# mkkellogg/GaussianSplats3D

Measured on AMD Instinct MI355X. Metric: Msplats/s sorted+rasterized at 1920x1080 SH-2, higher is better.
Workload: dtype int32 keys / f32 raster; 1 GPU; C3: garden.ply stand-in, SH2, 1920x1080; splats=5800000, sh_degree=2, width=1920, height=1080, cull=off (R=N), sort_precision_bits=16, streams=one (SURVEY.md 8d: sort -> draw on a single stream), parallelism=1 GPU, sort=full list (R = N)

## Files before the change

### gaussiansplats3d_amd/csrc/draw_plan.cpp

```cpp
#include "draw_plan.hpp"

#include "bin_word.hpp"

#include <math.h>
#include <string.h>

#include <algorithm>

DrawFeedback read_feedback(const volatile uint32_t* mirror) {
    DrawFeedback f = {};
    if (!mirror) return f;
    f.view_serial = mirror[GS_MIRROR_VIEW_SERIAL];
    f.visible = mirror[GS_MIRROR_VISIBLE];
    const uint32_t t_lo = mirror[GS_MIRROR_TILES16_LO], t_hi = mirror[GS_MIRROR_TILES16_HI];
    f.tiles16 = ((uint64_t)t_hi << 32) | t_lo;
    f.view_valid = f.view_serial != 0u && mirror[GS_MIRROR_VIEW_SERIAL] == f.view_serial;
    f.serial = mirror[GS_MIRROR_SERIAL];
    f.overflow = mirror[GS_MIRROR_OVERFLOW] != 0u;
    const uint32_t e_lo = mirror[GS_MIRROR_ENTRIES_LO], e_hi = mirror[GS_MIRROR_ENTRIES_HI];
    f.entries = ((uint64_t)e_hi << 32) | e_lo;
    f.entries_valid = mirror[GS_MIRROR_SERIAL] == f.serial;
    f.deep_candidates = mirror[GS_MIRROR_DEEP_CANDIDATES];
    f.deep_share = mirror[GS_MIRROR_DEEP_SHARE];
    return f;
}

uint32_t adapt_list_shift(uint32_t current, uint64_t tiles16, uint32_t visible) {
    if (visible == 0u) return current;
    const float tiles = (float)tiles16, vis = (float)visible;
    static const uint32_t shifts[4] = {GS_LIST_SHIFT_SMALL, GS_LIST_SHIFT_LARGE, GS_LIST_SHIFT_BIG, GS_LIST_SHIFT_HUGE};
    static const float thr[3] = {GS_LIST_TILES_PER_SPLAT, GS_LIST_TILES_PER_SPLAT_BIG, GS_LIST_TILES_PER_SPLAT_HUGE};
    uint32_t level = 0;
    while (level < 3u && shifts[level] != current) level++;
    while (level < 3u && tiles >= 1.08f * thr[level] * vis) level++;
    while (level > 0u && tiles < 0.92f * thr[level - 1u] * vis) level--;
    return shifts[level];
}

int block_test_mode(uint32_t measured_visible, uint32_t measured_count, bool strip, bool block_cull, bool no_block_list, bool block_test_always) {
    const bool measured = measured_count > 0u;
    const bool all_live = measured && (uint64_t)measured_visible * 10u > (uint64_t)measured_count * 9u;
    const bool half_live = measured && !all_live && (uint64_t)measured_visible * 20u > (uint64_t)measured_count * 11u;
    const bool test = block_cull && (!all_live || strip || block_test_always);
    const bool pretest = test && !no_block_list && (!half_live || strip || block_test_always);
    return pretest ? 1 : (test ? 0 : 2);
}

bool narrow_bin_word(uint32_t tiles_x, uint32_t tiles_y, const DrawSwitches& sw) {
    return tiles_x <= BIN_WORD_NARROW_TILES && tiles_y <= BIN_WORD_NARROW_TILES && !sw.no_compact_bin_word;
}

SchedulePlan plan_schedule(const ScheduleInputs& in) {
    const DrawSwitches& sw = in.sw;
    const PlanView& pp = in.now;
    SchedulePlan plan = {};
    const uint32_t blend_bins = in.bins_x * (in.bin_row_end - in.bin_row_begin);
    plan.blend_bins = blend_bins;
    plan.deep_factor = sw.deep_factor;
    plan.deep_min = in.draw_mode == GS_DRAW_FP32 ? sw.deep_min : 0x7FFFFFFFu;
    const bool order_ok = blend_bins > 0 && blend_bins <= 8192u && in.stats.bins == blend_bins && in.stats.row_begin == in.bin_row_begin &&
                          in.stats.width_px == (uint32_t)pp.width && in.stats.draw_mode == in.draw_mode && !sw.no_blend_order;
    plan.order_ok = order_ok;
    const PlanView& lp = in.stats.view;
    const bool same_frame = in.stats.valid && memcmp(lp.proj, pp.proj, sizeof(pp.proj)) == 0 && lp.width == pp.width && lp.height == pp.height &&
                            lp.count == pp.count && lp.list_shift == pp.list_shift;
    bool same_view = same_frame && memcmp(lp.view, pp.view, sizeof(pp.view)) == 0;
    if (same_frame && !same_view && in.block_cull && in.centre_n > 0) {
        const float limit = sw.order_motion;
        const double inv_n = 1.0 / (double)in.centre_n;
        const float c[3] = {(float)(in.centre_sum[0] * inv_n), (float)(in.centre_sum[1] * inv_n), (float)(in.centre_sum[2] * inv_n)};
        auto window = [&](const PlanView& q, const float* p, float* xy) {
            float v[4], o[4];
            for (int r = 0; r < 4; r++) v[r] = q.view[r] * p[0] + q.view[4 + r] * p[1] + q.view[8 + r] * p[2] + q.view[12 + r];
            for (int r = 0; r < 4; r++) o[r] = q.proj[r] * v[0] + q.proj[4 + r] * v[1] + q.proj[8 + r] * v[2] + q.proj[12 + r] * v[3];
            if (!(o[3] > 1e-6f)) return false;
            xy[0] = (o[0] / o[3] * 0.5f + 0.5f) * q.width;
            xy[1] = (o[1] / o[3] * 0.5f + 0.5f) * q.height;
            return true;
        };
        float was[2], is[2];
        if (window(lp, c, was) && window(pp, c, is)) {
            const float dx = (is[0] - was[0]) / (float)GS_BIN, dy = (is[1] - was[1]) / (float)GS_BIN;
            const bool shift_ok = fabsf(dx) < 4096.0f && fabsf(dy) < 4096.0f && !sw.no_stat_shift;
            if (shift_ok) {
                plan.sx = (int32_t)lrintf(dx);
                plan.sy = (int32_t)lrintf(dy);
            }
            const float* V = lp.view;
            const float a00 = V[0], a10 = V[1], a20 = V[2], a01 = V[4], a11 = V[5], a21 = V[6], a02 = V[8], a12 = V[9], a22 = V[10];
            const float c00 = a11 * a22 - a12 * a21, c01 = a02 * a21 - a01 * a22, c02 = a01 * a12 - a02 * a11;
            const float det = a00 * c00 + a10 * c01 + a20 * c02;
            const float b0 = V[12], b1 = V[13], b2 = V[14], id = 1.0f / det;
            const float eye[3] = {-(c00 * b0 + c01 * b1 + c02 * b2) * id,
                                  -((a12 * a20 - a10 * a22) * b0 + (a00 * a22 - a02 * a20) * b1 + (a02 * a10 - a00 * a12) * b2) * id,
                                  -((a10 * a21 - a11 * a20) * b0 + (a01 * a20 - a00 * a21) * b1 + (a00 * a11 - a01 * a10) * b2) * id};
            float parallax = 0.0f;
            bool seen = fabsf(det) > 1e-20f;
            for (int k = 0; k < 2 && seen; k++) {
                const float t = k ? 2.0f : 0.5f;
                const float p[3] = {eye[0] + t * (c[0] - eye[0]), eye[1] + t * (c[1] - eye[1]), eye[2] + t * (c[2] - eye[2])};
                float at[2];
                seen = window(pp, p, at);
                if (seen) parallax = fmaxf(parallax, sqrtf((at[0] - is[0]) * (at[0] - is[0]) + (at[1] - is[1]) * (at[1] - is[1])));
            }
            const float moved = (parallax + (shift_ok ? 0.0f : sqrtf(dx * dx + dy * dy) * (float)GS_BIN)) / fmaxf(pp.height, 1.0f);
            same_view = seen && moved <= limit;
        }
    }
    plan.same_view = same_view;
    const bool stale_order = sw.blend_order_stale;
    plan.deep_pass = order_ok && in.draw_mode == GS_DRAW_FP32 && !in.no_deep && in.feedback.deep_candidates > 0u;
    plan.order_wg = order_ok && (same_view || stale_order || plan.deep_pass || pp.list_shift == GS_LIST_SHIFT_SMALL || (in.draw_serial & 7u) == 7u);
    plan.order_taken = order_ok && (same_view || stale_order || (plan.deep_pass && !sw.deep_row_major_on_motion));
    return plan;
}

constexpr float DEEP_WGS_PER_SHARE = 0.6f;

DeepUnits place_deep_units(const SchedulePlan& plan, uint32_t bins, uint32_t cu_count, uint32_t occupancy, const DrawFeedback& feedback,
                           const DrawSwitches& sw) {
    DeepUnits du;
    du.unit_wgs = plan.deep_pass ? cu_count * occupancy : 0u;
    du.unit_at = bins;
    if (plan.deep_pass && plan.order_taken && !sw.deep_units_last) {
        const uint32_t cus = cu_count;
        const uint32_t deep_hint = feedback.deep_candidates;
        const float share = (float)std::min(feedback.deep_share, 1024u) * (1.0f / 1024.0f);
        const float k = DEEP_WGS_PER_SHARE;
        du.unit_wgs = std::min(du.unit_wgs, std::max(2u * cus, (uint32_t)(k * share * (float)du.unit_wgs + 0.5f)));
        du.unit_at = std::min(bins, std::min(deep_hint, (uint32_t)GS_DEEP_MAX_BINS) + cus + cus / 2u);
    }
    return du;
}

static PlanView plan_view(const float* view, const float* proj, float width, float height, uint32_t count, uint32_t list_shift) {
    PlanView v;
    memcpy(v.view, view, sizeof(v.view));
    memcpy(v.proj, proj, sizeof(v.proj));
    v.width = width; v.height = height; v.count = count; v.list_shift = list_shift;
    return v;
}

extern "C" int gs_debug_draw_plan(const gs_draw_plan_debug_in* in, gs_draw_plan_debug_out* out) {
    if (!in || !out) return -1;
    const DrawFeedback fb = read_feedback(in->mirror);
    ScheduleInputs si = {};
    si.stats.valid = in->stats_valid != 0u;
    si.stats.bins = in->stats_bins; si.stats.row_begin = in->stats_row_begin; si.stats.width_px = in->stats_width_px; si.stats.draw_mode = in->stats_mode;
    si.stats.view = plan_view(in->stats_view, in->stats_proj, in->stats_width, in->stats_height, in->stats_count, in->stats_list_shift);
    si.now = plan_view(in->view, in->proj, in->width, in->height, in->count, in->list_shift);
    si.bins_x = in->bins_x; si.bin_row_begin = in->bin_row_begin; si.bin_row_end = in->bin_row_end;
    si.block_cull = in->block_cull; si.draw_mode = in->draw_mode; si.draw_serial = in->draw_serial; si.no_deep = in->no_deep != 0u;
    memcpy(si.centre_sum, in->centre_sum, sizeof(si.centre_sum));
    si.centre_n = in->centre_n;
    si.feedback = fb;
    si.sw.deep_min = in->deep_min; si.sw.deep_factor = in->deep_factor; si.sw.no_blend_order = in->no_blend_order != 0u;
    si.sw.order_motion = in->order_motion; si.sw.no_stat_shift = in->no_stat_shift != 0u; si.sw.blend_order_stale = in->blend_order_stale != 0u;
    si.sw.deep_row_major_on_motion = in->deep_row_major_on_motion != 0u; si.sw.deep_units_last = in->deep_units_last != 0u;
    const SchedulePlan plan = plan_schedule(si);
    const DeepUnits du = place_deep_units(plan, plan.blend_bins, in->cu_count, in->occupancy, fb, si.sw);
    *out = gs_draw_plan_debug_out();
    out->entries = fb.entries; out->tiles16 = fb.tiles16; out->room = entry_room(in->need);
    out->entries_valid = fb.entries_valid; out->serial = fb.serial; out->overflow = fb.overflow;
    out->deep_candidates = fb.deep_candidates; out->deep_share = fb.deep_share;
    out->view_valid = fb.view_valid; out->view_serial = fb.view_serial; out->visible = fb.visible;
    out->blend_bins = plan.blend_bins; out->order_ok = plan.order_ok; out->same_view = plan.same_view;
    out->sx = plan.sx; out->sy = plan.sy;
    out->order_wg = plan.order_wg; out->order_taken = plan.order_taken; out->deep_pass = plan.deep_pass;
    out->deep_min = plan.deep_min; out->deep_factor = plan.deep_factor;
    out->unit_at = du.unit_at; out->unit_wgs = du.unit_wgs;
    out->list_shift = adapt_list_shift(in->list_current, in->tiles16, in->visible);
    out->block_test = block_test_mode(in->measured_visible, in->measured_count, in->strip != 0u, in->block_cull != 0u, in->no_block_list != 0u,
                                      in->block_test_always != 0u);
    return 0;
}

extern "C" int gs_debug_bin_word(const gs_bin_word_debug_in* in, gs_bin_word_debug_out* out) {
    if (!in || !out) return -1;
    DrawSwitches sw = {};
    sw.no_compact_bin_word = in->no_compact_bin_word != 0u;
    *out = gs_bin_word_debug_out();
    out->narrow = narrow_bin_word(in->tiles_x, in->tiles_y, sw) ? 1u : 0u;
    const BinRect r = {in->x0 | (in->y0 << 16), in->x1 | (in->y1 << 16)};
    out->word = bin_word_pack_narrow(in->visible != 0u, in->slot, r);
    const BinWordOut n = bin_word_unpack_narrow(out->word);
    out->visible = n.visible; out->escape = n.escape; out->slot = n.slot;
    if (n.visible && !n.escape) { out->x0 = n.rect.lo & 0xFFFFu; out->y0 = n.rect.lo >> 16; out->x1 = n.rect.hi & 0xFFFFu; out->y1 = n.rect.hi >> 16; }
    const BinWordWide w = bin_word_pack_wide(in->visible != 0u, in->slot, r);
    out->wide_lo = w.x; out->wide_hi = w.y;
    const BinWordOut u = bin_word_unpack_wide(w);
    out->wide_visible = u.visible; out->wide_slot = u.slot;
    out->wide_x0 = u.rect.lo & 0xFFFFu; out->wide_y0 = u.rect.lo >> 16; out->wide_x1 = u.rect.hi & 0xFFFFu; out->wide_y1 = u.rect.hi >> 16;
    return 0;
}
```

### gaussiansplats3d_amd/csrc/draw_plan.hpp

```cpp
#pragma once
#include <stdint.h>

#include "../../include/gsplat_hip.h"

constexpr uint32_t GS_BIN_SHIFT = 1;
constexpr uint32_t GS_BIN = GS_TILE << GS_BIN_SHIFT;
constexpr uint32_t GS_LIST_SHIFT_LARGE = 3;
constexpr uint32_t GS_LIST_SHIFT_SMALL = GS_BIN_SHIFT;
constexpr float GS_LIST_TILES_PER_SPLAT = 3.0f;
constexpr uint32_t GS_LIST_SHIFT_BIG = 4, GS_LIST_SHIFT_HUGE = 5;
constexpr float GS_LIST_TILES_PER_SPLAT_BIG = 21.0f, GS_LIST_TILES_PER_SPLAT_HUGE = 80.0f;
constexpr uint32_t GS_DEEP_MAX_BINS = 512;

constexpr uint32_t GS_MIRROR_SERIAL = 0, GS_MIRROR_OVERFLOW = 1, GS_MIRROR_ENTRIES_LO = 2, GS_MIRROR_ENTRIES_HI = 3;
constexpr uint32_t GS_MIRROR_DEEP_CANDIDATES = 4, GS_MIRROR_DEEP_SHARE = 5;
constexpr uint32_t GS_MIRROR_VIEW_SERIAL = 8, GS_MIRROR_VISIBLE = 9, GS_MIRROR_TILES16_LO = 10, GS_MIRROR_TILES16_HI = 11;
constexpr uint32_t GS_MIRROR_WORDS = 16;
static_assert(GS_MIRROR_SERIAL % 4 == 0 && GS_MIRROR_OVERFLOW == GS_MIRROR_SERIAL + 1 && GS_MIRROR_ENTRIES_LO == GS_MIRROR_SERIAL + 2 &&
              GS_MIRROR_ENTRIES_HI == GS_MIRROR_SERIAL + 3, "k_bin_emit writes the verdict as one aligned 16-byte store");
static_assert(GS_MIRROR_VIEW_SERIAL % 4 == 0 && GS_MIRROR_VISIBLE == GS_MIRROR_VIEW_SERIAL + 1 && GS_MIRROR_TILES16_LO == GS_MIRROR_VIEW_SERIAL + 2 &&
              GS_MIRROR_TILES16_HI == GS_MIRROR_VIEW_SERIAL + 3, "k_bin_emit writes the view share as one aligned 16-byte store");

struct DrawFeedback {
    bool entries_valid;
    uint32_t serial;
    bool overflow;
    uint64_t entries;
    uint32_t deep_candidates;
    uint32_t deep_share;
    bool view_valid;
    uint32_t view_serial, visible;
    uint64_t tiles16;
};
DrawFeedback read_feedback(const volatile uint32_t* mirror);

struct DrawSwitches {
    uint32_t deep_min;
    uint32_t deep_factor;
    uint32_t pool_slots;
    bool no_lazy_mask;
    bool no_blend_order;
    float order_motion;
    bool no_stat_shift;
    bool blend_order_stale;
    bool deep_row_major_on_motion;
    bool no_async_list_bins;
    bool deep_units_last;
    bool no_compact_bin_word;
};

uint32_t adapt_list_shift(uint32_t current, uint64_t tiles16, uint32_t visible);

inline uint64_t entry_room(uint64_t need) { return need + need / 8 + 1024; }

int block_test_mode(uint32_t measured_visible, uint32_t measured_count, bool strip, bool block_cull, bool no_block_list, bool block_test_always);

bool narrow_bin_word(uint32_t tiles_x, uint32_t tiles_y, const DrawSwitches& sw);

struct PlanView {
    float view[16], proj[16];
    float width, height;
    uint32_t count, list_shift;
};
struct StatsOf {
    bool valid;
    uint32_t bins, row_begin, width_px;
    uint32_t draw_mode;
    PlanView view;
};
struct ScheduleInputs {
    StatsOf stats;
    PlanView now;
    uint32_t bins_x, bin_row_begin, bin_row_end;
    uint32_t block_cull;
    uint32_t draw_mode;
    uint32_t draw_serial;
    bool no_deep;
    double centre_sum[3];
    uint64_t centre_n;
    DrawFeedback feedback;
    DrawSwitches sw;
};
struct SchedulePlan {
    uint32_t blend_bins;
    bool order_ok;
    bool same_view;
    int32_t sx, sy;
    bool order_wg;
    bool order_taken;
    bool deep_pass;
    uint32_t deep_min, deep_factor;
};
SchedulePlan plan_schedule(const ScheduleInputs& in);

struct DeepUnits { uint32_t unit_at, unit_wgs; };
DeepUnits place_deep_units(const SchedulePlan& plan, uint32_t bins, uint32_t cu_count, uint32_t occupancy, const DrawFeedback& feedback,
                           const DrawSwitches& sw);

struct gs_draw_plan_debug_in {
    double centre_sum[3];
    uint64_t centre_n;
    uint64_t tiles16;
    uint64_t need;
    uint32_t mirror[GS_MIRROR_WORDS];
    uint32_t stats_valid, stats_bins, stats_row_begin, stats_width_px, stats_mode;
    float stats_view[16], stats_proj[16], stats_width, stats_height;
    uint32_t stats_count, stats_list_shift;
    float view[16], proj[16], width, height;
    uint32_t count, list_shift, bins_x, bin_row_begin, bin_row_end, block_cull, draw_mode, draw_serial, no_deep;
    uint32_t deep_min, deep_factor, no_blend_order;
    float order_motion;
    uint32_t no_stat_shift, blend_order_stale, deep_row_major_on_motion, deep_units_last;
    uint32_t cu_count, occupancy;
    uint32_t list_current, visible;
    uint32_t measured_visible, measured_count, strip, no_block_list, block_test_always;
};
struct gs_draw_plan_debug_out {
    uint64_t entries, tiles16, room;
    uint32_t entries_valid, serial, overflow, deep_candidates, deep_share, view_valid, view_serial, visible;
    uint32_t blend_bins, order_ok, same_view;
    int32_t sx, sy;
    uint32_t order_wg, order_taken, deep_pass, deep_min, deep_factor;
    uint32_t unit_at, unit_wgs, list_shift;
    int32_t block_test;
};
extern "C" int gs_debug_draw_plan(const gs_draw_plan_debug_in* in, gs_draw_plan_debug_out* out);

struct gs_bin_word_debug_in {
    uint32_t tiles_x, tiles_y, no_compact_bin_word;
    uint32_t visible, slot, x0, y0, x1, y1;
};
struct gs_bin_word_debug_out {
    uint32_t narrow;
    uint32_t word;
    uint32_t visible, escape, slot, x0, y0, x1, y1;
    uint32_t wide_lo, wide_hi;
    uint32_t wide_visible, wide_slot, wide_x0, wide_y0, wide_x1, wide_y1;
};
extern "C" int gs_debug_bin_word(const gs_bin_word_debug_in* in, gs_bin_word_debug_out* out);
```

### gaussiansplats3d_amd/csrc/tile_bin.hip

```cpp
#include <stdlib.h>

#include "radix.hpp"

constexpr int BIN_THREADS = 256;
#ifndef BIN_PER_LANE
#define BIN_PER_LANE 4
#endif
#ifndef BIN_MAX_BLOCKS_CFG
#define BIN_MAX_BLOCKS_CFG 2048
#endif
constexpr int BIN_MAX_BLOCKS = BIN_MAX_BLOCKS_CFG;
constexpr uint32_t ANY_WORDS = 2048;

__device__ __forceinline__ uint32_t rect_tiles(uint2 r) {
    const uint32_t x0 = r.x & 0xFFFFu, y0 = r.x >> 16, x1 = r.y & 0xFFFFu, y1 = r.y >> 16;
    return (x1 >= x0 && y1 >= y0) ? (x1 - x0 + 1u) * (y1 - y0 + 1u) : 0u;
}
__device__ __forceinline__ uint2 rect_to_bins(uint2 r, uint32_t list_shift) {
    const uint32_t field = 0xFFFFu >> list_shift, mask = field | (field << 16);
    return make_uint2((r.x >> list_shift) & mask, (r.y >> list_shift) & mask);
}

struct BinChunk {
    uint32_t begin, end;
    uint32_t id;
};
__device__ __forceinline__ BinChunk bin_chunk(uint32_t n) {
    const uint32_t batches = (n + BIN_THREADS - 1) / BIN_THREADS;
    const uint32_t per = (batches + gridDim.x - 1) / gridDim.x;
    BinChunk c;
    c.id = xcd_chunk(blockIdx.x, gridDim.x);
    c.begin = min(c.id * per, batches);
    c.end = min(c.begin + per, batches);
    return c;
}

#ifdef GS_BIN_PROFILE
__device__ unsigned long long g_bin_prof[2 * 2048 * 4];
extern "C" int gs_debug_bin_prof(void* dst) {
    return (int)hipMemcpyFromSymbol(dst, HIP_SYMBOL(g_bin_prof), sizeof(unsigned long long) * 2 * 2048 * 4, 0, hipMemcpyDeviceToHost);
}
#define BIN_PROF(k, slot, v) do { if (threadIdx.x == 0 && blockIdx.x < 2048u) g_bin_prof[((k) * 2048 + blockIdx.x) * 4 + (slot)] = (v); } while (0)
#else
#define BIN_PROF(k, slot, v) do { } while (0)
#endif

struct SliceCount {
    uint32_t entries, splats, t16;
};
template <bool NARROW>
__device__ __forceinline__ SliceCount bin_count_slice(const uint32_t* __restrict__ order, uint32_t R, const uint32_t* __restrict__ perm,
                                                      const void* __restrict__ prect, const uint2* __restrict__ rects,
                                                      uint32_t* __restrict__ cidx, uint2* __restrict__ crect,
                                                      uint32_t* __restrict__ coff, uint32_t list_shift, uint32_t splat_count,
                                                      const uint8_t* __restrict__ block_any, bool coarse, const uint32_t* s_any,
                                                      unsigned long long* s_w, uint32_t pos_begin, uint32_t pos_end) {
    const uint32_t lane = threadIdx.x & 63u, wave = threadIdx.x >> 6;
    uint32_t sum = 0;
    uint32_t out = pos_begin;
    uint32_t t16 = 0;
    for (uint32_t pos0 = pos_begin; pos0 < pos_end; pos0 += BIN_PER_LANE * BIN_THREADS) {
        const uint32_t q0 = pos0 + (uint32_t)BIN_PER_LANE * threadIdx.x;
        uint32_t idx[BIN_PER_LANE];
        bool keep[BIN_PER_LANE];
        uint2 r[BIN_PER_LANE];
#pragma unroll
        for (int k = 0; k < BIN_PER_LANE; k++) {
            const uint32_t q = q0 + k;
            keep[k] = q < pos_end;
            const uint32_t p = R - 1u - min(q, R - 1u);
            idx[k] = order ? order[p] : p;
            keep[k] = keep[k] && idx[k] < splat_count;
            idx[k] = min(idx[k], splat_count - 1u);
        }
        if (perm) {
#pragma unroll
            for (int k = 0; k < BIN_PER_LANE; k++) idx[k] = perm[idx[k]];
        }
        if (coarse) {
#pragma unroll
            for (int k = 0; k < BIN_PER_LANE; k++) keep[k] = keep[k] && ((s_any[idx[k] >> 13] >> ((idx[k] >> 8) & 31u)) & 1u);
        } else if (block_any) {
#pragma unroll
            for (int k = 0; k < BIN_PER_LANE; k++) keep[k] = keep[k] && block_any[idx[k] >> 8] != 0;
        }
        uint32_t slot[BIN_PER_LANE];
        if (NARROW) {
            uint32_t w[BIN_PER_LANE];
#pragma unroll
            for (int k = 0; k < BIN_PER_LANE; k++) w[k] = keep[k] ? static_cast<const uint32_t*>(prect)[idx[k]] : BIN_WORD_INVISIBLE;
            bool esc[BIN_PER_LANE];
#pragma unroll
            for (int k = 0; k < BIN_PER_LANE; k++) {
                const BinWordOut o = bin_word_unpack_narrow(w[k]);
                keep[k] = o.visible;
                esc[k] = o.escape;
                slot[k] = (idx[k] & ~255u) + o.slot;
                r[k] = make_uint2(o.rect.lo, o.rect.hi);
            }
#pragma unroll
            for (int k = 0; k < BIN_PER_LANE; k++)
                if (esc[k]) r[k] = rects[slot[k]];
#pragma unroll
            for (int k = 0; k < BIN_PER_LANE; k++)
                if (!keep[k]) r[k] = make_uint2(0xFFFFu, 0u);
        } else {
#pragma unroll
            for (int k = 0; k < BIN_PER_LANE; k++) {
                const uint2 g = keep[k] ? static_cast<const uint2*>(prect)[idx[k]] : make_uint2(0u, 0u);
                const BinWordOut o = bin_word_unpack_wide(BinWordWide{g.x, g.y});
                keep[k] = keep[k] && o.visible;
                slot[k] = (idx[k] & ~255u) + o.slot;
                r[k] = keep[k] ? make_uint2(o.rect.lo, o.rect.hi) : make_uint2(0xFFFFu, 0u);
            }
        }
#pragma unroll
        for (int k = 0; k < BIN_PER_LANE; k++) t16 += rect_tiles(r[k]);
        uint32_t n[BIN_PER_LANE], cnt = 0, ent = 0;
#pragma unroll
        for (int k = 0; k < BIN_PER_LANE; k++) {
            n[k] = keep[k] ? rect_tiles(rect_to_bins(r[k], list_shift)) : 0u;
            cnt += keep[k] ? 1u : 0u;
            ent += n[k];
        }
        const unsigned long long mine = ((unsigned long long)cnt << 32) | ent;
        const unsigned long long incl = wave_incl_scan(mine, lane);
        if (lane == 63) s_w[wave] = incl;
        __syncthreads();
        unsigned long long base = 0, total = 0;
#pragma unroll
        for (int w = 0; w < 4; w++) {
            const unsigned long long c = s_w[w];
            base += ((uint32_t)w < wave) ? c : 0ull;
            total += c;
        }
        const unsigned long long excl = base + incl - mine;
        uint32_t o = out + (uint32_t)(excl >> 32);
        uint32_t e = sum + (uint32_t)excl;
#pragma unroll
        for (int k = 0; k < BIN_PER_LANE; k++) {
            if (keep[k]) {
                cidx[o] = slot[k];
                crect[o] = r[k];
                coff[o] = e;
                o++;
                e += n[k];
            }
        }
        out += (uint32_t)(total >> 32);
        sum += (uint32_t)total;
        __syncthreads();
    }
    SliceCount sc;
    sc.entries = sum; sc.splats = out - pos_begin; sc.t16 = t16;
    return sc;
}

template <bool NARROW>
__global__ __launch_bounds__(BIN_THREADS) __attribute__((amdgpu_waves_per_eu(8, 8))) void k_bin_count(const uint32_t* __restrict__ order, uint32_t R_host,
                                                           const uint32_t* __restrict__ R_dev ,
                                                           const uint32_t* __restrict__ perm,
                                                           const void* __restrict__ prect,
                                                           const uint2* __restrict__ rects ,
                                                           uint32_t* __restrict__ cidx,
                                                           uint2* __restrict__ crect, uint32_t* __restrict__ coff,
                                                           uint32_t* __restrict__ block_sums,
                                                           uint32_t* __restrict__ digit_total,
                                                           uint2* __restrict__ tile_ranges, uint32_t tiles, uint32_t list_shift,
                                                           uint32_t splat_count, const uint8_t* __restrict__ block_any,
                                                           uint32_t* __restrict__ deep_flags, uint32_t blend_bins,
                                                           uint32_t lds_bitmap ) {
    __shared__ unsigned long long s_w[4];
    __shared__ uint32_t s_any[ANY_WORDS];
    BIN_PROF(0, 0, wall_clock64());
    const uint32_t blocks = (splat_count + 255u) >> 8;
    const bool coarse = block_any != nullptr && blocks <= ANY_WORDS * 32u && lds_bitmap != 0u;
    if (coarse) {
        for (uint32_t w = threadIdx.x; w < (blocks + 31u) / 32u; w += BIN_THREADS) {
            const uint4* src = reinterpret_cast<const uint4*>(block_any + 32u * w);
            const uint4 a = src[0], b = src[1];
            const uint32_t v[8] = {a.x, a.y, a.z, a.w, b.x, b.y, b.z, b.w};
            uint32_t bits = 0;
#pragma unroll
            for (int k = 0; k < 8; k++)
                bits |= (((v[k] & 0xFFu) ? 1u : 0u) | ((v[k] & 0xFF00u) ? 2u : 0u) | ((v[k] & 0xFF0000u) ? 4u : 0u) |
                         ((v[k] & 0xFF000000u) ? 8u : 0u)) << (4 * k);
            s_any[w] = bits;
        }
        __syncthreads();
    }
    {
        const uint32_t t = blockIdx.x * BIN_THREADS + threadIdx.x, stride = gridDim.x * BIN_THREADS;
        for (uint32_t w = t; w < (uint32_t)RADIX_TOTAL_WORDS; w += stride) digit_total[w] = 0u;
        for (uint32_t w = t; w < tiles; w += stride) tile_ranges[w] = make_uint2(0xFFFFFFFFu, 0u);
        if (t < GS_FLAG_LIST) deep_flags[t] = 0u;
        for (uint32_t w = t; w < blend_bins; w += stride) deep_flags[GS_FLAG_OF + w] = GS_DEEP_NONE;
    }
    const uint32_t R = R_dev ? min(*R_dev, R_host) : R_host;
    const BinChunk ch = bin_chunk(R);
    BIN_PROF(0, 1, wall_clock64());
    if (blockIdx.x == 0 && threadIdx.x == 0) {
        const uint32_t batches = (R + BIN_THREADS - 1) / BIN_THREADS;
        block_sums[3 * BIN_MAX_BLOCKS] = (batches + gridDim.x - 1) / gridDim.x;
    }
    const uint32_t lane = threadIdx.x & 63u, wave = threadIdx.x >> 6;
    const uint32_t pos_begin = ch.begin * BIN_THREADS, pos_end = min(ch.end * BIN_THREADS, R);
    const SliceCount sc = bin_count_slice<NARROW>(order, R, perm, prect, rects, cidx, crect, coff, list_shift, splat_count, block_any, coarse, s_any, s_w, pos_begin, pos_end);
    uint32_t t16 = sc.t16;
    const uint32_t sum = sc.entries, out = pos_begin + sc.splats;
#pragma unroll
    for (int o = 32; o > 0; o >>= 1) t16 += __shfl_xor(t16, o, 64);
    if (lane == 0) s_w[wave] = t16;
    __syncthreads();
    if (threadIdx.x == 0) {
        block_sums[ch.id] = sum;
        block_sums[BIN_MAX_BLOCKS + ch.id] = out - pos_begin;
        block_sums[2 * BIN_MAX_BLOCKS + ch.id] = (uint32_t)(s_w[0] + s_w[1] + s_w[2] + s_w[3]);
    }
    BIN_PROF(0, 2, wall_clock64());
    BIN_PROF(0, 3, (unsigned long long)sum);
}

constexpr uint32_t EMIT_OWN = 16;
template <class KeyT>
__device__ __forceinline__ uint32_t bin_emit_batch(const uint32_t* __restrict__ cidx, const uint2* __restrict__ crect, const uint32_t* __restrict__ coff,
                                                   uint32_t src, bool live, uint32_t base, uint32_t limit, uint32_t tiles_x, uint32_t row_begin,
                                                   uint32_t list_shift, KeyT* __restrict__ keys_out, uint32_t* __restrict__ vals_out) {
    const uint32_t lane = threadIdx.x & 63u;
    auto put = [&](uint32_t e, uint32_t key, uint32_t idx) {
        if (e >= limit) return;
        keys_out[e] = (KeyT)key;
        vals_out[e] = idx;
    };
    uint2 r = make_uint2(0u, 0u);
    uint32_t idx = 0, e0 = 0, n = 0;
    if (live) {
        r = rect_to_bins(crect[src], list_shift);
        idx = cidx[src];
        e0 = base + coff[src];
        n = rect_tiles(r);
    }
    const uint32_t x0 = r.x & 0xFFFFu, y0 = r.x >> 16, w = (r.y & 0xFFFFu) - x0 + 1u;
    for (uint32_t k = 0, xx = x0, yy = y0; k < min(n, EMIT_OWN); k++) {
        put(e0 + k, (yy - row_begin) * tiles_x + xx, idx);
        if (++xx == x0 + w) { xx = x0; yy++; }
    }
    unsigned long long big = __ballot(n > EMIT_OWN);
    while (big) {
        const int sl = __builtin_ctzll(big);
        big &= big - 1ull;
        const uint32_t bn = __shfl(n, sl, 64), be0 = __shfl(e0, sl, 64), bidx = __shfl(idx, sl, 64);
        const uint32_t bx0 = __shfl(x0, sl, 64), by0 = __shfl(y0, sl, 64), bw = __shfl(w, sl, 64);
        const float inv_w = 1.0f / (float)bw;
        for (uint32_t k = EMIT_OWN + lane; k < bn; k += 64u) {
            uint32_t q = (uint32_t)((float)k * inv_w);
            int32_t rem = (int32_t)(k - q * bw);
            if (rem < 0) { q--; rem += (int32_t)bw; }
            else if (rem >= (int32_t)bw) { q++; rem -= (int32_t)bw; }
            put(be0 + k, (by0 + q - row_begin) * tiles_x + bx0 + (uint32_t)rem, bidx);
        }
    }
    return n;
}

struct StatShift {
    int32_t sx, sy;
    uint32_t bins_x;
};
__device__ __forceinline__ void blend_schedule_job(const uint2* prev_blend_stats, uint32_t blend_bins, uint32_t* __restrict__ blend_order,
                                                   uint32_t deep, uint32_t* __restrict__ deep_flags, uint32_t* blend_stats_w,
                                                   uint32_t deep_min, uint32_t deep_factor, volatile uint32_t* __restrict__ mirror, StatShift sh) {
    __shared__ uint32_t s_cost[RADIX_BINS], s_tmp2[4];
    constexpr uint32_t SWEEP = 8;
    auto cost_of = [&](uint32_t i) -> uint32_t {
        if (sh.sx == 0 && sh.sy == 0) return prev_blend_stats[i].y;
        const uint32_t by = i / sh.bins_x, bx = i - by * sh.bins_x;
        const int32_t fx = (int32_t)bx - sh.sx, fy = (int32_t)by - sh.sy;
        const uint32_t from = (uint32_t)fy * sh.bins_x + (uint32_t)fx;
        return (fx >= 0 && fy >= 0 && (uint32_t)fx < sh.bins_x && from < blend_bins) ? prev_blend_stats[from].y : 0u;
    };
    auto sweep = [&](auto&& use) {
        for (uint32_t base = 0; base < blend_bins; base += SWEEP * BIN_THREADS) {
            uint32_t c[SWEEP];
#pragma unroll
            for (uint32_t k = 0; k < SWEEP; k++) {
                const uint32_t i = base + threadIdx.x + k * BIN_THREADS;
                c[k] = i < blend_bins ? cost_of(i) : 0u;
            }
#pragma unroll
            for (uint32_t k = 0; k < SWEEP; k++) {
                const uint32_t i = base + threadIdx.x + k * BIN_THREADS;
                if (i < blend_bins) use(i, c[k]);
            }
        }
    };
    uint32_t sum = 0;
    sweep([&](uint32_t, uint32_t c) { sum += c; });
    uint32_t total_walked;
    (void)block_excl_scan_256(sum, s_tmp2, &total_walked);
    uint32_t shift = 0;
    while (((total_walked / blend_bins) >> shift) > 48u) shift++;
    s_cost[threadIdx.x] = 0u;
    __syncthreads();
    sweep([&](uint32_t, uint32_t c) { atomicAdd(&s_cost[255u - min(c >> shift, 255u)], 1u); });
    __syncthreads();
    const uint32_t cnt_d = s_cost[threadIdx.x];
    const uint32_t start = block_excl_scan_256(cnt_d, s_tmp2, nullptr);
    s_cost[threadIdx.x] = start;
    __syncthreads();
    sweep([&](uint32_t i, uint32_t c) { blend_order[atomicAdd(&s_cost[255u - min(c >> shift, 255u)], 1u)] = i; });
    const uint32_t mean_halves = total_walked / max(blend_bins, 1u);
    const uint32_t deep_trigger = max(2u * deep_min, deep_factor * mean_halves), deep_thr = max(2u * deep_min, mean_halves - mean_halves / 4u);
    __shared__ uint32_t s_trigger;
    if (threadIdx.x == 0) s_trigger = 0u;
    __shared__ uint32_t s_deep_n, s_deep_cost;
    if (threadIdx.x == 0) { s_deep_n = 0u; s_deep_cost = 0u; }
    __threadfence_block();
    __syncthreads();
    constexpr uint32_t HEAD_PER_T = (GS_DEEP_MAX_BINS + BIN_THREADS - 1u) / BIN_THREADS;
    uint32_t member[HEAD_PER_T];
#pragma unroll
    for (uint32_t q = 0; q < HEAD_PER_T; q++) {
        const uint32_t p = threadIdx.x + q * BIN_THREADS;
        member[q] = GS_DEEP_NONE;
        if (p >= min(blend_bins, GS_DEEP_MAX_BINS)) continue;
        const uint32_t i = __hip_atomic_load(&blend_order[p], __ATOMIC_RELAXED, __HIP_MEMORY_SCOPE_WORKGROUP);
        const uint32_t cost = i < blend_bins ? cost_of(i) : 0u;
        if (cost >= deep_trigger) s_trigger = 1u;
        if (cost >= deep_thr) {
            const uint32_t k = atomicAdd(&s_deep_n, 1u);
            atomicAdd(&s_deep_cost, cost >> 4);
            if (deep) {
                deep_flags[GS_FLAG_LIST + k] = i;
                deep_flags[GS_FLAG_OF + i] = k;
                member[q] = i;
            }
        }
    }
    __syncthreads();
#pragma unroll
    for (uint32_t q = 0; q < HEAD_PER_T; q++) {
        const uint32_t i = member[q];
        if (i != GS_DEEP_NONE) { blend_stats_w[2u * i] = 0u; blend_stats_w[2u * i + 1u] = 0u; blend_stats_w[2u * blend_bins + i] = 0u; }
    }
    if (threadIdx.x == 0) {
        deep_flags[GS_FLAG_CAND] = s_trigger ? s_deep_n : 0u;
        if (deep) deep_flags[GS_FLAG_COUNT] = s_deep_n;
        if (mirror) {
            mirror[GS_MIRROR_DEEP_CANDIDATES] = s_trigger ? s_deep_n : 0u;
            mirror[GS_MIRROR_DEEP_SHARE] = (uint32_t)(((unsigned long long)s_deep_cost << 14) / (unsigned long long)max(total_walked, 1u));
        }
    }
}

template <class KeyT>
__global__ __launch_bounds__(BIN_THREADS) void k_bin_emit(RenderFrame* __restrict__ frame, uint32_t capacity,
                                                          const uint32_t* __restrict__ cidx,
                                                          const uint2* __restrict__ crect, const uint32_t* __restrict__ coff,
                                                          const uint32_t* __restrict__ block_sums, uint32_t bin_grid,
                                                          uint32_t tiles_x ,
                                                          uint32_t row_begin , KeyT* __restrict__ keys_out,
                                                          uint32_t* __restrict__ vals_out, uint32_t list_shift,
                                                          volatile uint32_t* __restrict__ mirror, uint32_t serial,
                                                          const uint2* prev_blend_stats, uint32_t blend_bins,
                                                          uint32_t* __restrict__ blend_order, uint32_t deep,
                                                          uint32_t* __restrict__ deep_flags, uint32_t* blend_stats_w,
                                                          uint32_t deep_min, uint32_t deep_factor, StatShift sh) {
    __shared__ __attribute__((aligned(16))) uint32_t s_eoff[BIN_MAX_BLOCKS];
    __shared__ __attribute__((aligned(16))) uint32_t s_cnt[BIN_MAX_BLOCKS];
    __shared__ unsigned long long s_wsum[4], s_t16[4];
    __shared__ uint32_t s_vis[4];
    const uint32_t lane = threadIdx.x & 63u, wave = threadIdx.x >> 6;
    BIN_PROF(1, 0, wall_clock64());
    BIN_PROF(1, 2, 0ull);
    const uint32_t first_wg = blend_order ? 1u : 0u;
    if (blend_order && blockIdx.x == 0) {
        blend_schedule_job(prev_blend_stats, blend_bins, blend_order, deep, deep_flags, blend_stats_w, deep_min, deep_factor, mirror, sh);
        BIN_PROF(1, 1, wall_clock64());
        BIN_PROF(1, 2, wall_clock64());
        return;
    }
    const uint32_t wg = blockIdx.x - first_wg, wgs = gridDim.x - first_wg;
    constexpr uint32_t PER_T = BIN_MAX_BLOCKS / BIN_THREADS;
    static_assert(PER_T % 4 == 0, "16-byte loads of the workgroup sums");
    uint32_t mine[PER_T];
    unsigned long long own = 0;
#pragma unroll
    for (uint32_t q = 0; q < PER_T / 4; q++) {
        const uint32_t i0 = threadIdx.x * PER_T + 4 * q;
        const uint4 e = reinterpret_cast<const uint4*>(block_sums)[i0 / 4];
        uint4 c = reinterpret_cast<const uint4*>(block_sums + BIN_MAX_BLOCKS)[i0 / 4];
        mine[4 * q + 0] = i0 + 0 < bin_grid ? e.x : 0u;
        mine[4 * q + 1] = i0 + 1 < bin_grid ? e.y : 0u;
        mine[4 * q + 2] = i0 + 2 < bin_grid ? e.z : 0u;
        mine[4 * q + 3] = i0 + 3 < bin_grid ? e.w : 0u;
        c.x = i0 + 0 < bin_grid ? c.x : 0u;
        c.y = i0 + 1 < bin_grid ? c.y : 0u;
        c.z = i0 + 2 < bin_grid ? c.z : 0u;
        c.w = i0 + 3 < bin_grid ? c.w : 0u;
        reinterpret_cast<uint4*>(s_cnt)[i0 / 4] = c;
    }
#pragma unroll
    for (uint32_t k = 0; k < PER_T; k++) own += mine[k];
    const unsigned long long incl = wave_incl_scan(own, lane);
    if (lane == 63u) s_wsum[wave] = incl;
    __syncthreads();
    unsigned long long run = incl - own, D64 = 0;
#pragma unroll
    for (uint32_t w = 0; w < 4; w++) {
        const unsigned long long c = s_wsum[w];
        run += w < wave ? c : 0ull;
        D64 += c;
    }
#pragma unroll
    for (uint32_t q = 0; q < PER_T / 4; q++) {
        uint32_t v[4];
#pragma unroll
        for (uint32_t k = 0; k < 4; k++) {
            v[k] = run > 0xFFFFFFFFull ? 0xFFFFFFFFu : (uint32_t)run;
            run += mine[4 * q + k];
        }
        reinterpret_cast<uint4*>(s_eoff)[(threadIdx.x * PER_T + 4 * q) / 4] = make_uint4(v[0], v[1], v[2], v[3]);
    }
    const uint32_t D = D64 > capacity ? capacity : (uint32_t)D64;
    if (wg == 0) {
        unsigned long long t16 = 0;
        uint32_t vis = 0;
        for (uint32_t i = threadIdx.x; i < bin_grid; i += BIN_THREADS) {
            vis += block_sums[BIN_MAX_BLOCKS + i];
            t16 += block_sums[2 * BIN_MAX_BLOCKS + i];
        }
#pragma unroll
        for (int o = 32; o > 0; o >>= 1) {
            vis += __shfl_xor(vis, o, 64);
            t16 += __shfl_xor(t16, o, 64);
        }
        if (lane == 0u) { s_t16[wave] = t16; s_vis[wave] = vis; }
        __syncthreads();
        if (threadIdx.x == 0) {
            const unsigned long long tsum = s_t16[0] + s_t16[1] + s_t16[2] + s_t16[3];
            frame->tiles16_lo = (uint32_t)tsum;
            frame->tiles16_hi = (uint32_t)(tsum >> 32);
            frame->visible = s_vis[0] + s_vis[1] + s_vis[2] + s_vis[3];
            frame->entries_lo = (uint32_t)D64;
            frame->entries_hi = (uint32_t)(D64 >> 32);
            frame->overflow = D64 > capacity ? 1u : 0u;
            frame->entry_count = D;
            frame->pad = 0;
            if (mirror) {
                typedef uint32_t u32x4 __attribute__((ext_vector_type(4)));
                const u32x4 v = {serial, D64 > capacity ? 1u : 0u, (uint32_t)D64, (uint32_t)(D64 >> 32)};
                *reinterpret_cast<volatile u32x4*>(mirror + GS_MIRROR_SERIAL) = v;
                const u32x4 sv = {serial, s_vis[0] + s_vis[1] + s_vis[2] + s_vis[3], (uint32_t)tsum, (uint32_t)(tsum >> 32)};
                *reinterpret_cast<volatile u32x4*>(mirror + GS_MIRROR_VIEW_SERIAL) = sv;
            }
        }
    }
    __syncthreads();
    BIN_PROF(1, 1, wall_clock64());
    const uint32_t per = block_sums[3 * BIN_MAX_BLOCKS];
    const uint32_t units = bin_grid * per;
    uint32_t emitted = 0;
    for (uint32_t u = wg; u < units; u += wgs) {
        const uint32_t b = u / per, jb = (u - b * per) * BIN_THREADS;
        const uint32_t cnt = s_cnt[b], boff = s_eoff[b];
        if (jb >= cnt || boff >= D) continue;
        const uint32_t src = b * per * BIN_THREADS + jb + threadIdx.x;
        emitted += bin_emit_batch<KeyT>(cidx, crect, coff, src, jb + threadIdx.x < cnt, boff, D, tiles_x, row_begin, list_shift, keys_out, vals_out);
    }
    BIN_PROF(1, 2, wall_clock64());
    BIN_PROF(1, 3, (unsigned long long)emitted);
    (void)emitted;
}

static ScheduleInputs schedule_inputs(const gs_mesh* m, const DrawSwitches& sw, const DrawFeedback& fb, const ProjectParams& pp) {
    ScheduleInputs in;
    in.stats = m->stats_of;
    in.now = plan_view(pp);
    in.bins_x = pp.bins_x; in.bin_row_begin = pp.bin_row_begin; in.bin_row_end = pp.bin_row_end;
    in.block_cull = pp.block_cull;
    in.draw_mode = m->draw_mode;
    in.draw_serial = m->draw_serial;
    in.no_deep = m->no_deep;
    memcpy(in.centre_sum, m->centre_sum, sizeof(in.centre_sum));
    in.centre_n = m->centre_n;
    in.feedback = fb;
    in.sw = sw;
    return in;
}

template <class KeyT>
static int binning_typed(gs_mesh* m, const DrawSwitches& sw, const DrawFeedback& fb, const ProjectParams& pp, const uint32_t* order_dev, gs_sorter* sorter, uint32_t R, uint32_t tiles ) {
    gs_context* ctx = m->ctx;
    hipStream_t st = ctx->stream;
    const ProjSet& ps = m->set();
    const RadixExec ex = {st, &m->radix, ctx->lds_atomic_lane_order};
    RenderFrame* frame = m->frame.as<RenderFrame>();
    uint32_t grid = (R + BIN_THREADS - 1) / BIN_THREADS;
    if (grid < 1) grid = 1;
    if (grid > (uint32_t)BIN_MAX_BLOCKS) grid = BIN_MAX_BLOCKS;
    const uint32_t cap = m->entry_capacity;
    const uint32_t* R_dev = (sorter && sorter->last_plan.count_on_device) ? &sorter->result_frame->kept : nullptr;
    const uint32_t blend_bins = pp.bins_x * (pp.bin_row_end - pp.bin_row_begin);
    GS_TRY(m->deep_flags.ensure(((size_t)GS_FLAG_OF + blend_bins) * 4 + 64));
    GS_TRY(m->chunk_pool.ensure((size_t)GS_POOL_SLOTS * 256 * sizeof(float4)));
    GS_TRY(m->blend_stats.ensure((size_t)blend_bins * 12));
    if (sorter && sorter->stream != st) {
        GS_HIP(hipEventRecord(sorter->ev_consumed, st));
        sorter->consumer_pending = true;
    }
    m->plan = plan_schedule(schedule_inputs(m, sw, fb, pp));
    const SchedulePlan& plan = m->plan;
    if (plan.order_ok) GS_TRY(m->blend_order.ensure((size_t)blend_bins * 4));
    if (plan.deep_pass) {
        GS_TRY(m->deep_ent.ensure((size_t)GS_DEEP_MAX_BINS * GS_DEEP_LIST_CAP * 4));
        GS_TRY(m->deep_cnt.ensure((size_t)GS_DEEP_MAX_BINS * GS_DEEP_RANGES * 4 * 4));
        GS_TRY(m->deep_partial.ensure((size_t)GS_DEEP_UNITS * 256 * sizeof(float4)));
        GS_TRY(m->deep_work.ensure((size_t)GS_DEEP_UNITS * 4));
    }
    const bool order_wg = plan.order_wg;
    const StatShift stat_shift = {plan.sx, plan.sy, pp.bins_x};
    ++m->draw_serial;
    if (m->draw_serial == 0u) m->draw_serial = 1u;
    auto count_pass = [&](auto kernel) {
        hipLaunchKernelGGL(kernel, dim3(grid), dim3(BIN_THREADS), 0, st, order_dev, R, R_dev,
                           m->translate ? m->perm.as<uint32_t>() : nullptr, ps.prect.p, ps.rects.as<uint2>(), m->cidx.as<uint32_t>(), m->rect_q.as<uint2>(), m->coff.as<uint32_t>(),
                           m->bin_sums.as<uint32_t>(), m->radix.digit_total.as<uint32_t>(),
                           m->tile_ranges.as<uint2>(), tiles, pp.list_shift, pp.count,
                           ps.block_any.as<uint8_t>(), m->deep_flags.as<uint32_t>(), blend_bins, m->no_coarse_vis ? 0u : 1u);
    };
    if (ps.narrow_word) count_pass(k_bin_count<true>);
    else count_pass(k_bin_count<false>);
    hipLaunchKernelGGL((k_bin_emit<KeyT>), dim3(grid + (order_wg ? 1u : 0u)), dim3(BIN_THREADS), 0, st, frame, cap, m->cidx.as<uint32_t>(),
                       m->rect_q.as<uint2>(), m->coff.as<uint32_t>(), m->bin_sums.as<uint32_t>(), grid, pp.lists_x, pp.list_row_begin,
                       m->ekeyA.as<KeyT>(), m->evalA.as<uint32_t>(), pp.list_shift, m->mirror_dev, m->draw_serial,
                       order_wg ? m->blend_stats.as<uint2>() : nullptr, blend_bins, order_wg ? m->blend_order.as<uint32_t>() : nullptr,
                       plan.deep_pass ? 1u : 0u, m->deep_flags.as<uint32_t>(), m->blend_stats.as<uint32_t>(), plan.deep_min, plan.deep_factor, stat_shift);
    GS_HIP(hipGetLastError());
    if (pp.row_begin == 0u && pp.row_end >= pp.tiles_y) {
        m->full_serial[m->draw_serial & 7u] = m->draw_serial;
        m->full_count[m->draw_serial & 7u] = pp.count;
    }
    if (m->timed_draw) GS_HIP(hipEventRecord(m->ev[2], st));

    uint32_t bits = 1;
    while ((1ull << bits) < tiles) bits++;
    const uint32_t passes = (bits + 7) / 8;
    KeyT* kbuf[2] = {m->ekeyA.as<KeyT>(), m->ekeyB.as<KeyT>()};
    uint32_t* vbuf[2] = {m->evalA.as<uint32_t>(), m->evalB.as<uint32_t>()};
    for (uint32_t p = 0; p < passes; p++) {
        ArrayLoader<KeyT> al = {kbuf[p & 1], vbuf[p & 1], &frame->entry_count, 0u};
        if (passes == 1)
            GS_TRY((radix_pass<ArrayLoader<KeyT>, KeyT, false, false>(ex, al, al, cap, 0, 0, (KeyT*)nullptr, vbuf[1],
                                                                      m->tile_ranges.as<uint2>(), tiles)));
        else if (p + 1 == passes)
            GS_TRY((radix_pass<ArrayLoader<KeyT>, KeyT, false, true>(ex, al, al, cap, 8 * (int)p, (int)p, (KeyT*)nullptr,
                                                                     vbuf[(p + 1) & 1], m->tile_ranges.as<uint2>())));
        else
            GS_TRY((radix_pass<ArrayLoader<KeyT>, KeyT, true, false>(ex, al, al, cap, 8 * (int)p, (int)p, kbuf[(p + 1) & 1],
                                                                     vbuf[(p + 1) & 1])));
    }
    m->sorted_buf = (passes & 1);
    return GS_OK;
}

int gs_launch_binning(gs_mesh* m, const DrawSwitches& sw, const DrawFeedback& fb, const ProjectParams& pp, const uint32_t* order_dev, gs_sorter* sorter, uint32_t render_count) {
    const uint32_t tiles = pp.lists_x * (pp.list_row_end - pp.list_row_begin);
    if (tiles <= 65536u && !m->ctx->wide_entry_keys) return binning_typed<uint16_t>(m, sw, fb, pp, order_dev, sorter, render_count, tiles);
    return binning_typed<uint32_t>(m, sw, fb, pp, order_dev, sorter, render_count, tiles);
}
```

Measured before the change: 27310 Msplats/s.

## Compact emit loop over live batches with wave search and prefetched loads

The emit phase of k_bin_emit previously strode over every (slice, batch) pair and skipped empty ones. It now builds a per-slice packed word holding a prefix count of live batches. Each workgroup walks only live units, locating the slice with a two-level ballot search across the wave. The candidate loads for the next unit are issued before the current batch is emitted, so global-load latency overlaps the emit work. This adds an extra scan, a shared-memory array and search cost, and the 24-bit prefix field limits how many units can be encoded.

New measurement: 27730 Msplats/s (median of 6 runs). +1.6%, better.

```diff
diff --git a/gaussiansplats3d_amd/csrc/draw_plan.cpp b/gaussiansplats3d_amd/csrc/draw_plan.cpp
--- a/gaussiansplats3d_amd/csrc/draw_plan.cpp
+++ b/gaussiansplats3d_amd/csrc/draw_plan.cpp
@@ -6,6 +6,7 @@
 #include <string.h>
 
 #include <algorithm>
+#include <vector>
 
 DrawFeedback read_feedback(const volatile uint32_t* mirror) {
     DrawFeedback f = {};
@@ -193,3 +194,18 @@
     out->wide_x0 = u.rect.lo & 0xFFFFu; out->wide_y0 = u.rect.lo >> 16; out->wide_x1 = u.rect.hi & 0xFFFFu; out->wide_y1 = u.rect.hi >> 16;
     return 0;
 }
+
+extern "C" int64_t gs_debug_live_units(const uint32_t* cnt, uint32_t slices, uint32_t* units, uint32_t room) {
+    if (!cnt || slices == 0u || (!units && room != 0u)) return -1;
+    std::vector<uint32_t> words(slices);
+    uint32_t total = 0;
+    for (uint32_t b = 0; b < slices; b++) {
+        words[b] = live_unit_word(total, cnt[b]);
+        total += live_batches(cnt[b]);
+    }
+    for (uint32_t l = 0; l < std::min(total, room); l++) {
+        const LiveUnit u = live_unit_find([&](uint32_t b) { return words[b]; }, slices, total, l);
+        units[3u * l] = u.slice; units[3u * l + 1u] = u.batch; units[3u * l + 2u] = u.count;
+    }
+    return (int64_t)total;
+}
diff --git a/gaussiansplats3d_amd/csrc/draw_plan.hpp b/gaussiansplats3d_amd/csrc/draw_plan.hpp
--- a/gaussiansplats3d_amd/csrc/draw_plan.hpp
+++ b/gaussiansplats3d_amd/csrc/draw_plan.hpp
@@ -56,6 +56,38 @@
 int block_test_mode(uint32_t measured_visible, uint32_t measured_count, bool strip, bool block_cull, bool no_block_list, bool block_test_always);
 
 bool narrow_bin_word(uint32_t tiles_x, uint32_t tiles_y, const DrawSwitches& sw);
+
+#if defined(__HIP__)
+#define GS_PLAN_FN __attribute__((host)) __attribute__((device)) inline __attribute__((always_inline))
+#else
+#define GS_PLAN_FN inline
+#endif
+constexpr uint32_t GS_EMIT_BATCH = 256;
+constexpr uint32_t GS_LIVE_FIRST_MASK = 0x00FFFFFFu;
+GS_PLAN_FN uint32_t live_batches(uint32_t cnt) { return (cnt + GS_EMIT_BATCH - 1u) / GS_EMIT_BATCH; }
+GS_PLAN_FN uint32_t live_unit_word(uint32_t first, uint32_t cnt) { return (first & GS_LIVE_FIRST_MASK) | (((cnt - 1u) & 255u) << 24); }
+struct LiveUnit {
+    uint32_t slice, batch;
+    uint32_t count;
+};
+GS_PLAN_FN LiveUnit live_unit_of(uint32_t slice, uint32_t word, uint32_t next_first, uint32_t l) {
+    const uint32_t first = word & GS_LIVE_FIRST_MASK;
+    LiveUnit u;
+    u.slice = slice;
+    u.batch = l - first;
+    u.count = u.batch + 1u < next_first - first ? GS_EMIT_BATCH : (word >> 24) + 1u;
+    return u;
+}
+template <class WordAt>
+GS_PLAN_FN LiveUnit live_unit_find(WordAt word_at, uint32_t slices, uint32_t total, uint32_t l) {
+    uint32_t lo = 0u, hi = slices;
+    while (hi - lo > 1u) {
+        const uint32_t mid = (lo + hi) >> 1;
+        if ((word_at(mid) & GS_LIVE_FIRST_MASK) <= l) lo = mid;
+        else hi = mid;
+    }
+    return live_unit_of(lo, word_at(lo), hi < slices ? (word_at(hi) & GS_LIVE_FIRST_MASK) : total, l);
+}
 
 struct PlanView {
     float view[16], proj[16];
@@ -138,3 +170,5 @@
     uint32_t wide_visible, wide_slot, wide_x0, wide_y0, wide_x1, wide_y1;
 };
 extern "C" int gs_debug_bin_word(const gs_bin_word_debug_in* in, gs_bin_word_debug_out* out);
+
+extern "C" int64_t gs_debug_live_units(const uint32_t* cnt, uint32_t slices, uint32_t* units, uint32_t room);
diff --git a/gaussiansplats3d_amd/csrc/tile_bin.hip b/gaussiansplats3d_amd/csrc/tile_bin.hip
--- a/gaussiansplats3d_amd/csrc/tile_bin.hip
+++ b/gaussiansplats3d_amd/csrc/tile_bin.hip
@@ -221,10 +221,49 @@
     BIN_PROF(0, 3, (unsigned long long)sum);
 }
 
+struct EmitLoad {
+    bool live;
+    uint2 rect;
+    uint32_t idx, off, base;
+};
+constexpr uint32_t LIVE_BLOCK = 33;
+static_assert((uint32_t)BIN_MAX_BLOCKS <= 64u * LIVE_BLOCK, "one lane per block of slices");
+__device__ __forceinline__ LiveUnit live_unit_find_wave(const uint32_t* s_live, uint32_t slices, uint32_t total, uint32_t l) {
+    const uint32_t lane = threadIdx.x & 63u;
+    const uint32_t i1 = lane * LIVE_BLOCK;
+    const bool p1 = i1 < slices && (s_live[min(i1, slices - 1u)] & GS_LIVE_FIRST_MASK) <= l;
+    const uint32_t block = (uint32_t)__popcll(__ballot(p1)) - 1u;
+    const uint32_t i2 = block * LIVE_BLOCK + lane;
+    const bool mine = lane <= LIVE_BLOCK && i2 < slices;
+    const uint32_t w2 = mine ? s_live[min(i2, slices - 1u)] : 0u;
+    const bool p2 = mine && lane < LIVE_BLOCK && (w2 & GS_LIVE_FIRST_MASK) <= l;
+    const uint32_t in_block = (uint32_t)__popcll(__ballot(p2)) - 1u;
+    const uint32_t slice = block * LIVE_BLOCK + in_block;
+    const uint32_t word = __shfl(w2, (int)in_block, 64), after = __shfl(w2, (int)in_block + 1, 64);
+    return live_unit_of(slice, word, slice + 1u < slices ? (after & GS_LIVE_FIRST_MASK) : total, l);
+}
+
+__device__ __forceinline__ EmitLoad bin_emit_load(const uint32_t* __restrict__ cidx, const uint2* __restrict__ crect, const uint32_t* __restrict__ coff,
+                                                  const uint32_t* s_live, const uint32_t* s_eoff, uint32_t slices, uint32_t total, uint32_t per,
+                                                  uint32_t l, uint32_t limit) {
+    EmitLoad ld;
+    ld.live = false; ld.rect = make_uint2(0u, 0u); ld.idx = 0u; ld.off = 0u; ld.base = 0u;
+    if (l >= total) return ld;
+    const LiveUnit u = live_unit_find_wave(s_live, slices, total, l);
+    const uint32_t boff = s_eoff[u.slice];
+    if (boff >= limit || threadIdx.x >= u.count) return ld;
+    const uint32_t src = (u.slice * per + u.batch) * BIN_THREADS + threadIdx.x;
+    ld.live = true;
+    ld.rect = crect[src];
+    ld.idx = cidx[src];
+    ld.off = coff[src];
+    ld.base = boff;
+    return ld;
+}
+
 constexpr uint32_t EMIT_OWN = 16;
 template <class KeyT>
-__device__ __forceinline__ uint32_t bin_emit_batch(const uint32_t* __restrict__ cidx, const uint2* __restrict__ crect, const uint32_t* __restrict__ coff,
-                                                   uint32_t src, bool live, uint32_t base, uint32_t limit, uint32_t tiles_x, uint32_t row_begin,
+__device__ __forceinline__ uint32_t bin_emit_batch(const EmitLoad ld, uint32_t limit, uint32_t tiles_x, uint32_t row_begin,
                                                    uint32_t list_shift, KeyT* __restrict__ keys_out, uint32_t* __restrict__ vals_out) {
     const uint32_t lane = threadIdx.x & 63u;
     auto put = [&](uint32_t e, uint32_t key, uint32_t idx) {
@@ -232,14 +271,8 @@
         keys_out[e] = (KeyT)key;
         vals_out[e] = idx;
     };
-    uint2 r = make_uint2(0u, 0u);
-    uint32_t idx = 0, e0 = 0, n = 0;
-    if (live) {
-        r = rect_to_bins(crect[src], list_shift);
-        idx = cidx[src];
-        e0 = base + coff[src];
-        n = rect_tiles(r);
-    }
+    const uint2 r = rect_to_bins(ld.rect, list_shift);
+    const uint32_t idx = ld.idx, e0 = ld.base + ld.off, n = ld.live ? rect_tiles(r) : 0u;
     const uint32_t x0 = r.x & 0xFFFFu, y0 = r.x >> 16, w = (r.y & 0xFFFFu) - x0 + 1u;
     for (uint32_t k = 0, xx = x0, yy = y0; k < min(n, EMIT_OWN); k++) {
         put(e0 + k, (yy - row_begin) * tiles_x + xx, idx);
@@ -269,8 +302,9 @@
 };
 __device__ __forceinline__ void blend_schedule_job(const uint2* prev_blend_stats, uint32_t blend_bins, uint32_t* __restrict__ blend_order,
                                                    uint32_t deep, uint32_t* __restrict__ deep_flags, uint32_t* blend_stats_w,
-                                                   uint32_t deep_min, uint32_t deep_factor, volatile uint32_t* __restrict__ mirror, StatShift sh) {
-    __shared__ uint32_t s_cost[RADIX_BINS], s_tmp2[4];
+                                                   uint32_t deep_min, uint32_t deep_factor, volatile uint32_t* __restrict__ mirror, StatShift sh,
+                                                   uint32_t* s_tmp2 ) {
+    __shared__ uint32_t s_cost[RADIX_BINS];
     constexpr uint32_t SWEEP = 8;
     auto cost_of = [&](uint32_t i) -> uint32_t {
         if (sh.sx == 0 && sh.sy == 0) return prev_blend_stats[i].y;
@@ -367,15 +401,15 @@
                                                           uint32_t* __restrict__ deep_flags, uint32_t* blend_stats_w,
                                                           uint32_t deep_min, uint32_t deep_factor, StatShift sh) {
     __shared__ __attribute__((aligned(16))) uint32_t s_eoff[BIN_MAX_BLOCKS];
-    __shared__ __attribute__((aligned(16))) uint32_t s_cnt[BIN_MAX_BLOCKS];
+    __shared__ __attribute__((aligned(16))) uint32_t s_live[BIN_MAX_BLOCKS];
     __shared__ unsigned long long s_wsum[4], s_t16[4];
-    __shared__ uint32_t s_vis[4];
+    __shared__ uint32_t s_vis[4], s_lsum[4];
     const uint32_t lane = threadIdx.x & 63u, wave = threadIdx.x >> 6;
     BIN_PROF(1, 0, wall_clock64());
     BIN_PROF(1, 2, 0ull);
     const uint32_t first_wg = blend_order ? 1u : 0u;
     if (blend_order && blockIdx.x == 0) {
-        blend_schedule_job(prev_blend_stats, blend_bins, blend_order, deep, deep_flags, blend_stats_w, deep_min, deep_factor, mirror, sh);
+        blend_schedule_job(prev_blend_stats, blend_bins, blend_order, deep, deep_flags, blend_stats_w, deep_min, deep_factor, mirror, sh, s_lsum);
         BIN_PROF(1, 1, wall_clock64());
         BIN_PROF(1, 2, wall_clock64());
         return;
@@ -383,8 +417,9 @@
     const uint32_t wg = blockIdx.x - first_wg, wgs = gridDim.x - first_wg;
     constexpr uint32_t PER_T = BIN_MAX_BLOCKS / BIN_THREADS;
     static_assert(PER_T % 4 == 0, "16-byte loads of the workgroup sums");
-    uint32_t mine[PER_T];
+    uint32_t mine[PER_T], cnt[PER_T];
     unsigned long long own = 0;
+    uint32_t own_live = 0;
 #pragma unroll
     for (uint32_t q = 0; q < PER_T / 4; q++) {
         const uint32_t i0 = threadIdx.x * PER_T + 4 * q;
@@ -398,19 +433,24 @@
         c.y = i0 + 1 < bin_grid ? c.y : 0u;
         c.z = i0 + 2 < bin_grid ? c.z : 0u;
         c.w = i0 + 3 < bin_grid ? c.w : 0u;
-        reinterpret_cast<uint4*>(s_cnt)[i0 / 4] = c;
-    }
-#pragma unroll
-    for (uint32_t k = 0; k < PER_T; k++) own += mine[k];
+        cnt[4 * q + 0] = c.x; cnt[4 * q + 1] = c.y; cnt[4 * q + 2] = c.z; cnt[4 * q + 3] = c.w;
+    }
+#pragma unroll
+    for (uint32_t k = 0; k < PER_T; k++) { own += mine[k]; own_live += live_batches(cnt[k]); }
     const unsigned long long incl = wave_incl_scan(own, lane);
-    if (lane == 63u) s_wsum[wave] = incl;
+    const uint32_t incl_live = wave_incl_scan(own_live, lane);
+    if (lane == 63u) { s_wsum[wave] = incl; s_lsum[wave] = incl_live; }
     __syncthreads();
     unsigned long long run = incl - own, D64 = 0;
+    uint32_t run_live = incl_live - own_live, L = 0;
 #pragma unroll
     for (uint32_t w = 0; w < 4; w++) {
         const unsigned long long c = s_wsum[w];
         run += w < wave ? c : 0ull;
         D64 += c;
+        const uint32_t cl = s_lsum[w];
+        run_live += w < wave ? cl : 0u;
+        L += cl;
     }
 #pragma unroll
     for (uint32_t q = 0; q < PER_T / 4; q++) {
@@ -421,6 +461,12 @@
             run += mine[4 * q + k];
         }
         reinterpret_cast<uint4*>(s_eoff)[(threadIdx.x * PER_T + 4 * q) / 4] = make_uint4(v[0], v[1], v[2], v[3]);
+#pragma unroll
+        for (uint32_t k = 0; k < 4; k++) {
+            v[k] = live_unit_word(run_live, cnt[4 * q + k]);
+            run_live += live_batches(cnt[4 * q + k]);
+        }
+        reinterpret_cast<uint4*>(s_live)[(threadIdx.x * PER_T + 4 * q) / 4] = make_uint4(v[0], v[1], v[2], v[3]);
     }
     const uint32_t D = D64 > capacity ? capacity : (uint32_t)D64;
     if (wg == 0) {
@@ -459,18 +505,18 @@
     __syncthreads();
     BIN_PROF(1, 1, wall_clock64());
     const uint32_t per = block_sums[3 * BIN_MAX_BLOCKS];
-    const uint32_t units = bin_grid * per;
-    uint32_t emitted = 0;
-    for (uint32_t u = wg; u < units; u += wgs) {
-        const uint32_t b = u / per, jb = (u - b * per) * BIN_THREADS;
-        const uint32_t cnt = s_cnt[b], boff = s_eoff[b];
-        if (jb >= cnt || boff >= D) continue;
-        const uint32_t src = b * per * BIN_THREADS + jb + threadIdx.x;
-        emitted += bin_emit_batch<KeyT>(cidx, crect, coff, src, jb + threadIdx.x < cnt, boff, D, tiles_x, row_begin, list_shift, keys_out, vals_out);
+    uint32_t emitted = 0, walked = 0;
+    EmitLoad cur = bin_emit_load(cidx, crect, coff, s_live, s_eoff, bin_grid, L, per, wg, D);
+    __builtin_amdgcn_s_waitcnt(0x0F70);
+    for (uint32_t l = wg; l < L; l += wgs) {
+        const EmitLoad next = bin_emit_load(cidx, crect, coff, s_live, s_eoff, bin_grid, L, per, l + wgs, D);
+        emitted += bin_emit_batch<KeyT>(cur, D, tiles_x, row_begin, list_shift, keys_out, vals_out);
+        cur = next;
+        walked++;
     }
     BIN_PROF(1, 2, wall_clock64());
-    BIN_PROF(1, 3, (unsigned long long)emitted);
-    (void)emitted;
+    BIN_PROF(1, 3, (unsigned long long)emitted | ((unsigned long long)walked << 32));
+    (void)emitted; (void)walked;
 }
 
 static ScheduleInputs schedule_inputs(const gs_mesh* m, const DrawSwitches& sw, const DrawFeedback& fb, const ProjectParams& pp) {
```
